# flock-lab/flock

Hardware: AMD Instinct MI355X
Metric: NEXMark rows/sec per node (q3 join, q5 agg) (higher is better)
Workload: dtype int32; 1 GPU; NEXMark q5 hopping(10,5) over 1087 s x 1000000 events/s per GPU; query=q5, input_rows_per_gpu=1000040000, windows_per_gpu=216, parallelism=one GPU, one process

## Files before the change

flock_amd/csrc/q5.hip:

```cpp
#include <algorithm>

#include "sort.hpp"

using namespace flockgpu;

namespace {

constexpr int kQ5Iters = 8;
constexpr int kQ5Tile = kBlock * 4 * kQ5Iters;
constexpr int kHist = 4096;
constexpr int kHistPad = 64;
constexpr int kSlots = kHist / 2;
constexpr int kSlotBits = 11;
static_assert(kSlots == (1 << kSlotBits), "slot bits");
constexpr int kLdsMaxProbe = 24;
constexpr uint32_t kFib = 0x9E3779B1u;
constexpr int kHotMin = 16;
constexpr int kMaxWinPanes = 8;
constexpr uint32_t kWideTile = 0x40000000u;

using u16x2 = unsigned short __attribute__((ext_vector_type(2)));
__device__ __forceinline__ u16x2 as_u16x2(uint32_t w) { return __builtin_bit_cast(u16x2, w); }
__device__ __forceinline__ u16x2 nonzero_u16x2(u16x2 c) {
    uint32_t r;
// ... 95 lines not shown
        const int32_t w = f.pane_win_idx[wi];
        table_add(f.tables + (size_t)w * f.cap, f.cap, (uint32_t)key, c, &f.tab_used[w], f.err);
    }
}

__device__ __forceinline__ void emit_pair16(int32_t even_key, uint32_t c0, uint32_t c1, const FlushArgs &f) {
    const uint64_t idx = (uint64_t)((int64_t)even_key - f.pane.base);
    if (idx < (uint64_t)f.pane.range) {
        __hip_atomic_fetch_add(&f.counters[(f.pane.cnt_off + idx) >> 1], c0 | (c1 << 16), __ATOMIC_RELAXED, __HIP_MEMORY_SCOPE_AGENT);
        return;
    }
    if (c0) emit_pair(even_key, c0, f);
    if (c1) emit_pair(even_key + 1, c1, f);
}

constexpr int kRangeBlocks = 2;
__global__ __launch_bounds__(kBlock) void q5_range_kernel(const int32_t *__restrict__ auction, int64_t n_rows,
                                                          const int64_t *__restrict__ seg_off, int32_t *__restrict__ rng) {
    __shared__ int32_t s_red[8];
    const int32_t pane = blockIdx.y;
    const int64_t sb = seg_off[2 * pane], se = seg_off[2 * pane + 1];
    const int64_t groups = (se - (sb & ~int64_t(3)) + 3) >> 2;
    const int64_t n_samples = (int64_t)kRangeBlocks * kBlock * 4;
    const int64_t stride = groups > n_samples ? groups / n_samples : 1;
    int32_t mn = 0x7fffffff, mx = (int32_t)0x80000000;
#pragma unroll
    for (int i = 0; i < 4; ++i) {
        const int64_t g = ((int64_t)(i * kRangeBlocks + blockIdx.x) * kBlock + threadIdx.x) * stride;
        const int64_t r0 = (sb & ~int64_t(3)) + g * 4;
        if (g < groups && r0 + 4 <= n_rows) {
            const int4 t = *reinterpret_cast<const int4 *>(auction + r0);
            const int32_t k[4] = {t.x, t.y, t.z, t.w};
#pragma unroll
            for (int j = 0; j < 4; ++j)
                if (r0 + j >= sb && r0 + j < se) {
                    mn = min(mn, k[j]);
                    mx = max(mx, k[j]);
                }
        }
    }
#pragma unroll
    for (int o = 32; o > 0; o >>= 1) {
        mn = min(mn, __shfl_xor(mn, o, 64));
        mx = max(mx, __shfl_xor(mx, o, 64));
    }
    if (lane_id() == 0) {
        s_red[threadIdx.x >> 6] = mn;
        s_red[4 + (threadIdx.x >> 6)] = mx;
    }
    __syncthreads();
    if (threadIdx.x == 0) {
        int32_t *o = rng + ((size_t)pane * kRangeBlocks + blockIdx.x) * 2;
        o[0] = min(min(s_red[0], s_red[1]), min(s_red[2], s_red[3]));
        o[1] = max(max(s_red[4], s_red[5]), max(s_red[6], s_red[7]));
    }
}

__host__ __device__ inline bool q5_pane_layout(int64_t lo, int64_t hi, int64_t *base, int64_t *range) {
    const int64_t span = hi - lo, margin = span / 16 > 4096 ? span / 16 : 4096;
    *base = (lo - margin) & ~int64_t(7);
    *range = ((hi + margin + 1 - *base) + 7) & ~int64_t(7);
    return *range < (int64_t(1) << 31);
}

struct LayoutArgs {
    const int32_t *rng;
    const int32_t *pane_win_ptr;
    const int64_t *seg_off;
    int32_t n_panes, n_win;
    uint64_t capacity, budget_bytes;
    PaneDesc *panes;
    WinDesc *wins;
    uint64_t *info;
};
__device__ __forceinline__ void q5_layout_block(const int32_t *__restrict__ rng, const int32_t *__restrict__ pane_win_ptr,
                                                const int64_t *__restrict__ seg_off, int32_t n_panes, int32_t n_win,
                                                uint64_t capacity, uint64_t budget_bytes, PaneDesc *__restrict__ panes,
                                                WinDesc *__restrict__ wins, uint64_t *__restrict__ info) {
    __shared__ uint64_t s_wave[kWavesPerBlock];
    __shared__ uint64_t s_carry;
    __shared__ int s_ok;
    const int lane = lane_id(), wave = threadIdx.x >> 6;
    if (threadIdx.x == 0) {
        s_carry = 0;
        s_ok = 1;
    }
    __syncthreads();
    for (int32_t p0 = 0; p0 < n_panes; p0 += kBlock) {
        const int32_t p = p0 + (int32_t)threadIdx.x;
        int64_t base = 0, range = 0;
        if (p < n_panes && pane_win_ptr[p + 1] != pane_win_ptr[p] && seg_off[2 * p + 1] > seg_off[2 * p]) {
            int32_t mn = 0x7fffffff, mx = (int32_t)0x80000000;
            for (int b = 0; b < kRangeBlocks; ++b) {
                mn = min(mn, rng[((size_t)p * kRangeBlocks + b) * 2]);
                mx = max(mx, rng[((size_t)p * kRangeBlocks + b) * 2 + 1]);
            }
            if (mn <= mx && !q5_pane_layout(mn, mx, &base, &range)) {
                s_ok = 0;
                range = 0;
            }
        }
        const uint64_t incl = wave_incl_scan_u64((uint64_t)range);
        if (lane == 63) s_wave[wave] = incl;
        __syncthreads();
        uint64_t off = s_carry + incl - (uint64_t)range;
        for (int v = 0; v < wave; ++v) off += s_wave[v];
        if (p < n_panes) panes[p] = PaneDesc{base, off, (uint32_t)range, 0};
        __syncthreads();
        if (threadIdx.x == kBlock - 1) s_carry = off + (uint64_t)range;
        __syncthreads();
    }
    const uint64_t cnt_total = s_carry;
    __syncthreads();
    uint64_t scan = 0;
    for (int32_t w = threadIdx.x; w < n_win; w += kBlock) {
        WinDesc d = wins[w];
// ... 15 lines not shown
                scan += (uint64_t)(hi - lo);
            }
        }
        wins[w] = d;
    }
    scan = wave_sum_u64(scan);
    if (lane == 0) s_wave[wave] = scan;
    __syncthreads();
    if (threadIdx.x == 0) {
        uint64_t scan_total = 0;
        for (int v = 0; v < kWavesPerBlock; ++v) scan_total += s_wave[v];
        const bool ok = s_ok && cnt_total <= capacity && cnt_total * 4 <= budget_bytes && scan_total * 4 <= 2 * budget_bytes;
        info[0] = cnt_total;
        info[1] = scan_total;
        info[2] = ok ? 1 : 0;
    }
}

__global__ __launch_bounds__(kBlock) void q5_clear_kernel(uint32_t *__restrict__ counters, uint64_t cnt_host,
                                                          uint64_t cnt_from, uint64_t *__restrict__ tables, uint64_t table_words,
                                                          uint64_t *__restrict__ meta, uint64_t meta_words, int32_t *__restrict__ slow_list,
                                                          uint32_t *__restrict__ block_max, uint64_t block_max_words, int c16, LayoutArgs lay,
                                                          const uint64_t *__restrict__ cnt_info) {
    if (lay.rng && blockIdx.x == 0) q5_layout_block(lay.rng, lay.pane_win_ptr, lay.seg_off, lay.n_panes, lay.n_win, lay.capacity, lay.budget_bytes, lay.panes, lay.wins, lay.info);
    uint64_t cnt = cnt_host;
    if (cnt_info) cnt = cnt_info[2] ? (cnt_info[0] < cnt_host ? cnt_info[0] : cnt_host) : 0;
    if (c16) cnt = (cnt + 1) / 2;
    const uint64_t i0 = (uint64_t)blockIdx.x * kBlock + threadIdx.x, stride = (uint64_t)gridDim.x * kBlock;
    const uint4 z = make_uint4(0, 0, 0, 0);
    for (uint64_t i = i0 + cnt_from / 4; i * 4 < cnt + 3; i += stride) {
        uint32_t *p = counters + i * 4;
        __builtin_nontemporal_store(0u, p);
        __builtin_nontemporal_store(0u, p + 1);
        __builtin_nontemporal_store(0u, p + 2);
        __builtin_nontemporal_store(0u, p + 3);
    }
    for (uint64_t i = i0; i * 2 < table_words; i += stride) {
        if (i * 2 + 1 < table_words) reinterpret_cast<uint4 *>(tables)[i] = z;
        else tables[i * 2] = 0;
    }
// ... 706 lines not shown
            uint64_t t = 0;
#pragma unroll
            for (int v = 0; v < kWavesPerBlock; ++v) t += s_groups[2][v];
            if (t) atomicAdd(&pane_sum[p], (unsigned long long)t);
        }
    }
}

constexpr int kFinishThreads = 1024;
constexpr uint32_t kFinishMax = 1024;
__global__ __launch_bounds__(kFinishThreads) void q5_finish_kernel(const uint64_t *__restrict__ meta, uint32_t n_meta, int32_t n_win, const uint64_t *__restrict__ info,
                                                                   const int32_t *__restrict__ slow_list, const int32_t *__restrict__ sel_win,
                                                                   const int32_t *__restrict__ sel_key, uint32_t out_cap, int32_t *__restrict__ out_auction,
                                                                   uint64_t *__restrict__ out_num, uint64_t *__restrict__ h_fin,
                                                                   const unsigned long long *__restrict__ pane_sum, const unsigned long long *__restrict__ tab_rows,
                                                                   const int64_t *__restrict__ seg_off, const int32_t *__restrict__ pane_win_ptr, int32_t n_panes) {
    __shared__ uint64_t s_k[kFinishMax];
    __shared__ uint32_t s_bad;
    const uint32_t *tail = reinterpret_cast<const uint32_t *>(meta + 2 * (size_t)n_win);
    const uint32_t n_sel = tail[0], err = tail[1];
    if (threadIdx.x == 0) s_bad = 0;
    __syncthreads();
    if (pane_sum && (!info || info[2]))
        for (int32_t p = threadIdx.x; p < n_panes; p += kFinishThreads)
            if (pane_win_ptr[p + 1] != pane_win_ptr[p] && pane_sum[p] + tab_rows[p] != (unsigned long long)(seg_off[2 * p + 1] - seg_off[2 * p])) s_bad = 1;
    __syncthreads();
    const uint32_t bad16 = s_bad;
    for (uint32_t i = threadIdx.x; i < n_meta; i += kFinishThreads) h_fin[i] = meta[i];
    if (threadIdx.x < 3) h_fin[n_meta + threadIdx.x] = info ? info[threadIdx.x] : 0;
    if (threadIdx.x == 3) h_fin[n_meta + 3] = (uint64_t)(uint32_t)slow_list[0] | ((uint64_t)bad16 << 32);
    const bool sortable = !err && !bad16 && n_sel <= kFinishMax && n_sel <= out_cap && (!info || info[2]);
    if (threadIdx.x == 4) h_fin[n_meta + 4] = sortable ? 1 : 0;
    int64_t *h_off = reinterpret_cast<int64_t *>(h_fin + n_meta + 5);
    if (!sortable) return;
    uint32_t p2 = 1;
    while (p2 < n_sel) p2 <<= 1;
    if (threadIdx.x < p2)
        s_k[threadIdx.x] = threadIdx.x < n_sel ? ((uint64_t)(uint32_t)sel_win[threadIdx.x] << 32) | ((uint32_t)sel_key[threadIdx.x] ^ 0x80000000u) : ~0ull;
    __syncthreads();
    for (uint32_t k = 2; k <= p2; k <<= 1)
        for (uint32_t j = k >> 1; j > 0; j >>= 1) {
            const uint32_t i = threadIdx.x, l = i ^ j;
            if (i < p2 && l > i) {
                const uint64_t a = s_k[i], b = s_k[l];
// ... 351 lines not shown
        now.insert(now.end(), idx.begin(), idx.end());
        if (sig != now) {
            std::copy(ptr.begin(), ptr.end(), h_ptr);
            std::copy(idx.begin(), idx.end(), h_idx);
            std::copy(role_a.begin(), role_a.end(), h_roles);
            std::copy(role_b.begin(), role_b.end(), h_roles + role_a.size());
            FG_HIP(ctx, hipMemcpyAsync(d_ptr, h_ptr, ptr.size() * sizeof(int32_t), hipMemcpyHostToDevice, ctx->stream));
            if (!idx.empty())
                FG_HIP(ctx, hipMemcpyAsync(d_idx, h_idx, idx.size() * sizeof(int32_t), hipMemcpyHostToDevice, ctx->stream));
            FG_HIP(ctx, hipMemcpyAsync(d_roles, h_roles, 2 * role_a.size() * sizeof(int32_t), hipMemcpyHostToDevice, ctx->stream));
            sig = now;
        }
    }

    int32_t *d_rng = nullptr, *h_rng = nullptr;
    const size_t n_rng = (size_t)2 * kRangeBlocks * std::max(n_panes, 1);
    FG_TRY(arena_get_t(ctx, "q5.pane_range", n_rng + 2, &d_rng));
    FG_TRY(pinned_get_t(ctx, "q5.pane_range", n_rng + 2, &h_rng));
    std::vector<PaneDesc> panes((size_t)std::max(n_panes, 1));
    std::vector<WinDesc> wins((size_t)std::max(n_win, 1));
    for (auto &p : panes) p = PaneDesc{0, 0, 0, 0};
    for (int w = 0; w < n_win; ++w) wins[w] = WinDesc{0, 0, win->win_pane_lo[w], win->win_pane_hi[w], 0};
    uint64_t cnt_total = 0, scan_total = 0;
    bool dense = st.n_tiles > 0 && n_win > 0 && max_win_panes <= kMaxWinPanes;
    std::vector<int64_t> &hint = ctx->host_i64[weight ? "q5.layout_hint.weighted" : "q5.layout_hint"];
    if (hint.size() != 3) hint.assign(3, 0);
    const uint64_t budget = std::max<uint64_t>(uint64_t(256) << 20, (uint64_t)covered_rows * 4 * 2);
    if (dense) {
        LaunchScope ls(ctx, "q5_range_kernel");
        hipLaunchKernelGGL(q5_range_kernel, dim3(kRangeBlocks, (unsigned)n_panes), dim3(kBlock), 0, ctx->stream, auction, rows, st.seg_off, d_rng);
    }
    FG_TRY(check_launch(ctx, "q5_range_kernel"));
    std::vector<int64_t> &wide_hint = ctx->host_i64["q5.wide_hint"];
    if (wide_hint.size() != 1) wide_hint.assign(1, 0);
    bool wide_mode = wide_hint[0] != 0 && !weight && !part && dense;
    bool wide_ran = false;
    bool speculate = dense && !part && hint[2] && hint[0] > 0 && !wide_mode;
    auto host_layout = [&]() -> int {
        FG_HIP(ctx, hipMemcpyAsync(h_rng, d_rng, sizeof(int32_t) * n_rng, hipMemcpyDeviceToHost, ctx->stream));
        FG_HIP(ctx, hipStreamSynchronize(ctx->stream));
        cnt_total = scan_total = 0;
        for (int p = 0; p < n_panes && dense; ++p) {
            if (ptr[p + 1] == ptr[p] || se[p] <= sb[p]) continue;
            int64_t lo = INT64_MAX, hi = INT64_MIN;
            for (int b = 0; b < kRangeBlocks; ++b) {
                lo = std::min<int64_t>(lo, h_rng[((size_t)p * kRangeBlocks + b) * 2]);
                hi = std::max<int64_t>(hi, h_rng[((size_t)p * kRangeBlocks + b) * 2 + 1]);
            }
            if (lo > hi) continue;
            int64_t base = 0, range = 0;
            if (!q5_pane_layout(lo, hi, &base, &range)) { dense = false; break; }
            panes[p] = PaneDesc{base, cnt_total, (uint32_t)range, 0};
            cnt_total += (uint64_t)range;
        }
        for (int w = 0; w < n_win && dense; ++w) {
            int64_t lo = INT64_MAX, hi = INT64_MIN;
            for (int p = win->win_pane_lo[w]; p < win->win_pane_hi[w]; ++p)
                if (panes[p].range) {
                    lo = std::min(lo, panes[p].base);
                    hi = std::max(hi, panes[p].base + (int64_t)panes[p].range);
                }
            if (lo >= hi) continue;
            if (hi - lo >= (int64_t(1) << 31)) { dense = false; break; }
            wins[w].base = lo;
            wins[w].range = (uint32_t)(hi - lo);
            scan_total += (uint64_t)(hi - lo);
        }
        if (dense && (cnt_total * 4 > budget || scan_total * 4 > 2 * budget)) dense = false;
        return FLOCKGPU_OK;
    };
    if (dense && !speculate) FG_TRY(host_layout());
    PaneDesc *d_panes = nullptr, *h_panes = nullptr;
    WinDesc *d_wins = nullptr, *h_wins = nullptr;
    FG_TRY(arena_get_t(ctx, "q5.panes", panes.size(), &d_panes));
    FG_TRY(pinned_get_t(ctx, "q5.panes", panes.size(), &h_panes));
    FG_TRY(arena_get_t(ctx, "q5.wins", wins.size(), &d_wins));
    FG_TRY(pinned_get_t(ctx, "q5.wins", wins.size(), &h_wins));
    uint64_t *d_info = nullptr, *h_info = nullptr;
    FG_TRY(arena_get_t(ctx, "q5.layout_info", 4, &d_info));
    FG_TRY(pinned_get_t(ctx, "q5.layout_info", 4, &h_info));
    auto upload_layout = [&]() -> int {
        if (!dense) {
            cnt_total = scan_total = 0;
            for (auto &p : panes) p = PaneDesc{0, 0, 0, 0};
            for (int w = 0; w < n_win; ++w) wins[w] = WinDesc{0, 0, win->win_pane_lo[w], win->win_pane_hi[w], 0};
        }
        std::copy(panes.begin(), panes.end(), h_panes);
        std::copy(wins.begin(), wins.end(), h_wins);
        ctx->host_i64["q5.wins_sig"].clear();
        FG_HIP(ctx, hipMemcpyAsync(d_panes, h_panes, panes.size() * sizeof(PaneDesc), hipMemcpyHostToDevice, ctx->stream));
        FG_HIP(ctx, hipMemcpyAsync(d_wins, h_wins, wins.size() * sizeof(WinDesc), hipMemcpyHostToDevice, ctx->stream));
        return FLOCKGPU_OK;
    };
    uint32_t *counters = nullptr;
    uint64_t capacity = 0;
    std::vector<int64_t> &preclean = ctx->host_i64["q5.preclean"];
    if (preclean.size() != 2) preclean.assign(2, 0);
    LayoutArgs lay{};
    uint64_t clean_upto = 0;
    const bool c16 = !weight && !part && !wide_mode && hop2 && ctx->host_i64["q5.no_c16"].empty();
    auto words_of = [&](uint64_t n_counters) -> uint64_t { return c16 ? (n_counters + 1) / 2 : n_counters; };
    if (speculate) {
        FG_TRY(arena_get_t(ctx, "q5.counters", (size_t)words_of((uint64_t)hint[0] + (uint64_t)hint[0] / 8) + 8, &counters));
        capacity = (ctx->arena["q5.counters"].cap / sizeof(uint32_t) - 8) * (c16 ? 2 : 1);
        if (preclean[0] == (int64_t)reinterpret_cast<uintptr_t>(counters)) clean_upto = (uint64_t)preclean[1];
        {
            std::vector<int64_t> &wsig = ctx->host_i64["q5.wins_sig"];
            std::vector<int64_t> wnow;
            wnow.reserve((size_t)2 * n_win + 2);
            wnow.push_back((int64_t)reinterpret_cast<uintptr_t>(d_wins));
            for (int w = 0; w < n_win; ++w) {
                wnow.push_back(win->win_pane_lo[w]);
                wnow.push_back(win->win_pane_hi[w]);
            }
            if (wsig != wnow) {
                std::copy(wins.begin(), wins.end(), h_wins);
                FG_HIP(ctx, hipMemcpyAsync(d_wins, h_wins, wins.size() * sizeof(WinDesc), hipMemcpyHostToDevice, ctx->stream));
                wsig = wnow;
            }
        }
// ... 18 lines not shown
    if (weight && n_panes > 0) {
        FG_TRY(arena_get_t(ctx, "q5.pane_weight", (size_t)n_panes + 1, &d_wsum));
        FG_TRY(pinned_get_t(ctx, "q5.pane_weight", (size_t)n_panes + 1, &h_wsum));
    }
    double rpg = ctx->q5_rows_per_group < 1.0 ? 1.0 : ctx->q5_rows_per_group;
    uint64_t cap64 = dense ? 1024 : std::max<uint64_t>(1024, (uint64_t)((double)max_win_rows / rpg * 2.0) + 64);
    uint32_t out_cap = 1u << 16;
    std::vector<int32_t> h_win, h_key;
    uint32_t n_sel = 0;
    const int32_t *sel_win = nullptr, *sel_key = nullptr;
    bool fin_sorted = false;
    const int64_t *fin_off = nullptr;
    const int32_t *fin_auction = nullptr;
    const uint64_t *fin_num = nullptr;
    uint32_t h_slow_count = 0;
    for (int attempt = 0;; ++attempt) {
        if (attempt > 8 || cap64 >= (uint64_t(1) << 31))
            return fail(ctx, FLOCKGPU_ERR_CAPACITY, "q5: hash table capacity %llu still overflows", (unsigned long long)cap64);
        const uint32_t cap = (uint32_t)cap64;
        const uint64_t *spec_info = speculate ? d_info : nullptr;
        uint64_t *tables = nullptr;
        FG_TRY(arena_get_t(ctx, "q5.tables", (size_t)cap * std::max(n_win, 1), &tables));
        int32_t *o_win = nullptr, *o_key = nullptr, *slow_list = nullptr;
        FG_TRY(arena_get_t(ctx, "q5.sel_win", out_cap, &o_win));
        FG_TRY(arena_get_t(ctx, "q5.sel_key", out_cap, &o_key));
        FG_TRY(arena_get_t(ctx, "q5.slow_list", (size_t)st.n_tiles + 2, &slow_list));
        const uint64_t per_win = n_win > 0 ? std::max<uint64_t>(cap, scan_total / n_win / 4) : cap;
        const bool pane_walk = hop2;
        const uint64_t per_pane = n_panes > 0 ? std::max<uint64_t>(cap, cnt_total / (uint64_t)n_panes / 4) : cap;
        const int hop2_blocks = c16 ? 16 : 32;
        const unsigned gx = (unsigned)std::min<int64_t>(std::max<int64_t>(div_up((int64_t)(pane_walk ? per_pane : per_win), kBlock * 2), 1), pane_walk ? hop2_blocks : 64);
        uint32_t *block_max = nullptr;
        const uint64_t n_block_max = (uint64_t)gx * std::max(n_win, 1) * (pane_walk ? 2 : 1);
        FG_TRY(arena_get_t(ctx, "q5.block_max", (size_t)n_block_max, &block_max));
        {
            const uint64_t clear_words = std::max<uint64_t>({words_of(speculate ? capacity : cnt_total), (uint64_t)cap * n_win, (uint64_t)n_meta_all, n_block_max});
            const unsigned cg = (unsigned)std::max<int64_t>(1, std::min<int64_t>(div_up((int64_t)clear_words / 4 + 1, kBlock), (int64_t)ctx->num_cus * 16));
            {
                LaunchScope ls(ctx, "q5_clear_kernel");
                hipLaunchKernelGGL(q5_clear_kernel, dim3(cg), dim3(kBlock), 0, ctx->stream, counters, speculate ? capacity : cnt_total,
                                   (attempt == 0 && speculate) ? (clean_upto & ~uint64_t(3)) : uint64_t(0), tables, (uint64_t)cap * n_win, d_meta, (uint64_t)n_meta_all,
                                   slow_list, block_max, n_block_max, c16 ? 1 : 0, speculate ? lay : LayoutArgs{}, (const uint64_t *)nullptr);
                if (speculate) clean_upto = std::max(clean_upto, words_of(capacity));
            }
            FG_TRY(check_launch(ctx, "q5_clear_kernel"));
        }
        if (d_wsum) FG_HIP(ctx, hipMemsetAsync(d_wsum, 0, sizeof(unsigned long long) * (size_t)n_panes, ctx->stream));
        uint32_t nd = 0;
        if (wide_mode && dense) {
            uint32_t max_range = 0;
            for (int p = 0; p < n_panes; ++p) max_range = std::max(max_range, panes[(size_t)p].range);
            nd = (uint32_t)div_up((int64_t)max_range, int64_t(1) << kPartShift) + 1;
        }
        const bool wide = wide_mode && dense && nd >= 2 && nd <= (uint32_t)kPartMaxDigits && st.n_tiles > 0 && n_win > 0;
        wide_ran = wide;
        uint32_t *d_sample = nullptr, *h_sample = nullptr;
        FG_TRY(arena_get_t(ctx, "q5.part_sample", 4, &d_sample));
// ... 20 lines not shown
                LaunchScope ls(ctx, "q5_bucket_count_kernel");
                hipLaunchKernelGGL(q5_bucket_count_kernel, dim3(nd, (unsigned)n_panes), dim3(kBlock), 0, ctx->stream, part_keys, part_low, st4, d_panes, d_ptr, d_idx, nd,
                                   off_mat, counters, tables, cap, d_used, d_err);
            }
            FG_TRY(check_launch(ctx, "q5_bucket_count_kernel"));
            FG_HIP(ctx, hipMemcpyAsync(h_sample, d_sample, 2 * sizeof(uint32_t), hipMemcpyDeviceToHost, ctx->stream));
        } else if (st.n_tiles > 0 && n_win > 0) {
            {
                LaunchScope ls(ctx, "q5_count_kernel");
                hipLaunchKernelGGL(weight ? q5_count_kernel<true> : q5_count_kernel<false>, dim3((unsigned)st.n_tiles), dim3(kBlock), 0,
                                   ctx->stream, auction, weight, st, d_panes, d_ptr, d_idx, counters, tables, cap, d_used, d_err,
                                   slow_list, spec_info, d_wsum, c16 ? 1 : 0, c16 ? d_tab_rows : (unsigned long long *)nullptr);
            }
            FG_TRY(check_launch(ctx, "q5_count_kernel"));
            if (d_wsum) FG_HIP(ctx, hipMemcpyAsync(h_wsum, d_wsum, sizeof(unsigned long long) * (size_t)n_panes, hipMemcpyDeviceToHost, ctx->stream));
            {
                LaunchScope ls(ctx, "q5_count_slow_kernel");
                const unsigned gs = (unsigned)std::min<int64_t>(st.n_tiles, (int64_t)ctx->num_cus * 8);
                hipLaunchKernelGGL(weight ? q5_count_slow_kernel<true> : q5_count_slow_kernel<false>, dim3(gs), dim3(kBlock), 0,
                                   ctx->stream, auction, weight, st, d_panes, d_ptr, d_idx, counters, tables, cap, d_used, d_err,
                                   slow_list, spec_info, c16 ? 1 : 0, c16 ? d_tab_rows : (unsigned long long *)nullptr);
            }
            FG_TRY(check_launch(ctx, "q5_count_slow_kernel"));
        }
        if (part) {
            const int64_t tab0 = ((int64_t)cnt_total + 3) & ~int64_t(3);
            std::vector<int64_t> xb((size_t)2 * n_win), xe((size_t)2 * n_win);
            for (int w = 0; w < n_win; ++w) {
                xb[2 * w] = (int64_t)panes[w].cnt_off;
                xe[2 * w] = (int64_t)panes[w].cnt_off + (int64_t)panes[w].range;
                xb[2 * w + 1] = tab0 + (int64_t)w * cap;
// ... 73 lines not shown
            }
            FG_TRY(check_launch(ctx, "q5_select_kernel"));
        }
        constexpr uint32_t kSpecWinners = 4096;
        uint64_t *h_fin = nullptr;
        int32_t *fin_a = nullptr;
        uint64_t *fin_n = nullptr;
        FG_TRY(pinned_get_t(ctx, "q5.finish", n_meta + 8 + (size_t)n_win + 2, &h_fin));
        FG_TRY(arena_get_t(ctx, "q5.out_auction", (size_t)kFinishMax + 1, &fin_a));
        FG_TRY(arena_get_t(ctx, "q5.out_num", (size_t)kFinishMax + 1, &fin_n));
        const bool poll = !d_wsum && !wide;
        if (poll) pinned_pending(h_fin, (int)(n_meta + 5 + (size_t)n_win + 1));
        {
            LaunchScope ls(ctx, "q5_finish_kernel");
            hipLaunchKernelGGL(q5_finish_kernel, dim3(1), dim3(kFinishThreads), 0, ctx->stream, d_meta, (uint32_t)n_meta, n_win, spec_info, slow_list, o_win, o_key, out_cap,
                               fin_a, fin_n, h_fin, c16 && pane_walk ? d_pane_sum : (const unsigned long long *)nullptr, d_tab_rows, st.seg_off, d_ptr, n_panes);
        }
        FG_TRY(check_launch(ctx, "q5_finish_kernel"));
        if (speculate && dense) {
            LaunchScope ls(ctx, "q5_clear_kernel");
            const unsigned cg = (unsigned)std::max<int64_t>(1, std::min<int64_t>(div_up((int64_t)words_of(cnt_total) / 4 + 1, kBlock), (int64_t)ctx->num_cus * 16));
            hipLaunchKernelGGL(q5_clear_kernel, dim3(cg), dim3(kBlock), 0, ctx->stream, counters, capacity, uint64_t(0), (uint64_t *)nullptr,
                               uint64_t(0), (uint64_t *)nullptr, uint64_t(0), slow_list, (uint32_t *)nullptr, uint64_t(0), c16 ? 1 : 0, LayoutArgs{}, d_info);
        }
        FG_TRY(check_launch(ctx, "q5_clear_kernel"));
        if (poll) {
            FG_TRY(wait_pinned(ctx, h_fin, (int)(n_meta + 5)));
            if (h_fin[n_meta + 4]) FG_TRY(wait_pinned(ctx, h_fin + n_meta + 5, n_win + 1));
        } else
            FG_HIP(ctx, hipStreamSynchronize(ctx->stream));
        std::copy(h_fin, h_fin + n_meta, h_meta);
        if (speculate) std::copy(h_fin + n_meta, h_fin + n_meta + 3, h_info);
        h_slow_count = (uint32_t)h_fin[n_meta + 3];
        if (h_fin[n_meta + 3] >> 32) {
            ctx->host_i64["q5.no_c16"].assign(1, 1);
            return q5_run(ctx, auction, weight, rows, win, out, part);
        }
        fin_sorted = h_fin[n_meta + 4] != 0;
        fin_off = reinterpret_cast<const int64_t *>(h_fin + n_meta + 5);
        if (speculate) {
            if (!h_info[2]) {
                speculate = false;
                hint[2] = 0;
                FG_TRY(host_layout());
                FG_TRY(upload_layout());
                FG_TRY(arena_get_t(ctx, "q5.counters", (size_t)words_of(cnt_total) + 8, &counters));
                cap64 = dense ? 1024 : std::max<uint64_t>(1024, (uint64_t)((double)max_win_rows / rpg * 2.0) + 64);
                --attempt;
                continue;
            }
            cnt_total = h_info[0];
            scan_total = h_info[1];
        }
        if (h_wsum) {
            for (int w = 0; w < n_win; ++w) {
                unsigned long long tot = 0;
                for (int p = win->win_pane_lo[w]; p < win->win_pane_hi[w]; ++p) tot += h_wsum[p];
                if (tot >= (1ull << 32))
                    return fail(ctx, FLOCKGPU_ERR_UNSUPPORTED, "q5 weighted: the counts of window %d add up to %llu >= 2^32 (32-bit counters)", w, tot);
            }
        }
        const uint32_t *tail = reinterpret_cast<const uint32_t *>(h_meta + 2 * n_win);
        n_sel = tail[0];
        if (tail[1]) {
            cap64 *= 4;
            continue;
        }
// ... 4 lines not shown
        h_win.resize(n_sel);
        h_key.resize(n_sel);
        if (fin_sorted) {
            fin_auction = fin_a;
            fin_num = fin_n;
        } else if (n_sel <= kSpecWinners) {
            FG_HIP(ctx, hipMemcpyAsync(h_win.data(), o_win, sizeof(int32_t) * n_sel, hipMemcpyDeviceToHost, ctx->stream));
            FG_HIP(ctx, hipMemcpyAsync(h_key.data(), o_key, sizeof(int32_t) * n_sel, hipMemcpyDeviceToHost, ctx->stream));
            FG_HIP(ctx, hipStreamSynchronize(ctx->stream));
        } else {
            sel_win = o_win;
            sel_key = o_key;
        }
        break;
    }
    hint[0] = (int64_t)cnt_total;
    hint[1] = (int64_t)scan_total;
    hint[2] = dense ? 1 : 0;
    if (!weight && !part) {
        uint32_t *h_sample = nullptr;
        FG_TRY(pinned_get_t(ctx, "q5.part_sample", 4, &h_sample));
        if (wide_mode && !wide_ran) wide_hint[0] = 0;
        else if (wide_mode && h_sample[0]) wide_hint[0] = (uint64_t)h_sample[1] * 4 >= (uint64_t)h_sample[0] * 3 ? 0 : 1;
        else if (!wide_mode && dense && st.n_tiles > 64) wide_hint[0] = (int64_t)h_slow_count * 4 > (int64_t)st.n_tiles ? 1 : 0;
    }
    {
        double best = 1e30;
        for (int w = 0; w < n_win; ++w) {
            const int64_t rows = win->pane_row_offsets[win->win_pane_hi[w]] - win->pane_row_offsets[win->win_pane_lo[w]];
            const uint64_t g = h_meta[n_win + w];
            if (g) best = std::min(best, (double)rows / (double)g);
        }
        if (best < 1e30) ctx->q5_rows_per_group = best;
    }
    std::vector<int64_t> &offs = ctx->host_i64["q5.win_out_offsets"];
    std::vector<uint64_t> &wmax = ctx->host_u64["q5.win_max"], &wgrp = ctx->host_u64["q5.win_groups"];
    offs.assign((size_t)n_win + 1, 0);
    wmax.assign(h_meta, h_meta + n_win);
    wgrp.assign(h_meta + n_win, h_meta + 2 * n_win);
// ... 16 lines not shown
        FG_TRY(key_min_max(ctx, sel_key, n_sel, d_mm));
        FG_HIP(ctx, hipMemcpyAsync(h_mm, d_mm, 2 * sizeof(int32_t), hipMemcpyDeviceToHost, ctx->stream));
        FG_HIP(ctx, hipStreamSynchronize(ctx->stream));
        int bits = 1, wbits = 1;
        while (bits < 32 && (((uint64_t)((int64_t)h_mm[1] - (int64_t)h_mm[0])) >> bits)) ++bits;
        while (wbits < 31 && ((uint32_t)n_win >> wbits)) ++wbits;
        FG_TRY(radix_sort_pairs(ctx, "q5.ord_key", sel_key, nullptr, n_sel, h_mm[0], bits, &k1, &v1));
        FG_TRY(arena_get_t(ctx, "q5.ord_win_in", (size_t)n_sel + 4, &w_in));
        FG_TRY(gather_i32(ctx, sel_win, reinterpret_cast<const int32_t *>(v1), n_sel, w_in));
        FG_TRY(radix_sort_pairs(ctx, "q5.ord_win", w_in, v1, n_sel, 0, wbits, &w2, &v2));
        FG_TRY(arena_get_t(ctx, "q5.out_auction", (size_t)n_sel + 1, &d_oa));
        FG_TRY(arena_get_t(ctx, "q5.out_num", (size_t)n_sel + 1, &d_on));
        FG_TRY(arena_get_t(ctx, "q5.ord_off", (size_t)n_win + 2, &d_off));
        FG_TRY(pinned_get_t(ctx, "q5.ord_off", (size_t)n_win + 2, &h_off));
        FG_TRY(gather_i32(ctx, sel_key, reinterpret_cast<const int32_t *>(v2), n_sel, d_oa));
        hipLaunchKernelGGL(q5_winner_num_kernel, dim3((unsigned)div_up((int64_t)n_sel, kBlock)), dim3(kBlock), 0, ctx->stream, w2,
                           d_meta, (int64_t)n_sel, d_on);
        FG_TRY(check_launch(ctx, "q5_winner_num_kernel"));
        FG_TRY(sorted_key_offsets(ctx, w2, n_sel, n_win, d_off));
        FG_HIP(ctx, hipMemcpyAsync(h_off, d_off, sizeof(int64_t) * ((size_t)n_win + 1), hipMemcpyDeviceToHost, ctx->stream));
        FG_HIP(ctx, hipStreamSynchronize(ctx->stream));
        offs.assign(h_off, h_off + n_win + 1);
        out->auction = d_oa;
        out->num = d_on;
        out->win_out_offsets = offs.data();
        out->win_max = wmax.data();
        out->win_groups = wgrp.data();
        out->rows = n_sel;
        return FLOCKGPU_OK;
    }
// ... 19 lines not shown
    FG_TRY(arena_get_t(ctx, "q5.out_auction", (size_t)n_sel + 1, &d_oa));
    FG_TRY(arena_get_t(ctx, "q5.out_num", (size_t)n_sel + 1, &d_on));
    if (n_sel) {
        FG_HIP(ctx, hipMemcpyAsync(d_oa, h_oa, sizeof(int32_t) * n_sel, hipMemcpyHostToDevice, ctx->stream));
        FG_HIP(ctx, hipMemcpyAsync(d_on, h_on, sizeof(uint64_t) * n_sel, hipMemcpyHostToDevice, ctx->stream));
    }
    out->auction = d_oa;
    out->num = d_on;
    out->win_out_offsets = offs.data();
    out->win_max = wmax.data();
    out->win_groups = wgrp.data();
    out->rows = n_sel;
    }
    if (speculate && dense && cnt_total > 0) {
        preclean[0] = (int64_t)reinterpret_cast<uintptr_t>(counters);
        preclean[1] = (int64_t)std::max<uint64_t>(clean_upto, words_of(cnt_total));
    }
    return FLOCKGPU_OK;
}

namespace flockgpu {

int q5_partial_by_tile(flockgpu_ctx *ctx, const flockgpu_bid_cols *bid, const flockgpu_windows *win, Q5TilePartial *out) {
    *out = Q5TilePartial{};
    FG_TRY(check_windows(ctx, win, bid->rows, "q5 partial"));
    if (bid->rows > 0 && !bid->auction) return fail(ctx, FLOCKGPU_ERR_INVALID, "q5 partial: null auction column");
    if (reinterpret_cast<uintptr_t>(bid->auction) & 15) return fail(ctx, FLOCKGPU_ERR_UNSUPPORTED, "q5: auction column must be 16-byte aligned");
    if (bid->rows >= (int64_t(1) << 31)) return fail(ctx, FLOCKGPU_ERR_UNSUPPORTED, "q5 partial: more than 2^31 rows per call");
    FG_HIP(ctx, hipSetDevice(ctx->device));
    const int n_panes = win->n_panes;
    std::vector<char> used((size_t)std::max(n_panes, 1), 0);
// ... 83 lines not shown
```

Baseline: 1351 billion rows/s.

## Use fixed per-pane counter slots with in-kernel layout and skip redundant clears

The range kernel now runs one 1024-thread block per pane, computes each pane's layout descriptor on the device, and assigns fixed-size counter slots sized from a remembered max pane range. On steady repeated calls this lets the path skip the full clear/layout kernel. The post-finish clear runs per pane, and the slow-path count kernel is skipped unless slow tiles were seen recently. The goal is to cut per-call launch, clear and layout overhead. The cost is much more complex state tracking across calls, with a retry if skipped slow work turns out to be needed.

```diff
diff --git a/flock_amd/csrc/q5.hip b/flock_amd/csrc/q5.hip
--- a/flock_amd/csrc/q5.hip
+++ b/flock_amd/csrc/q5.hip
@@ -133,23 +133,44 @@
     if (c1) emit_pair(even_key + 1, c1, f);
 }
 
+__host__ __device__ inline bool q5_pane_layout(int64_t lo, int64_t hi, int64_t *base, int64_t *range) {
+    const int64_t span = hi - lo, margin = span / 16 > 4096 ? span / 16 : 4096;
+    *base = (lo - margin) & ~int64_t(7);
+    *range = ((hi + margin + 1 - *base) + 7) & ~int64_t(7);
+    return *range < (int64_t(1) << 31);
+}
+
 constexpr int kRangeBlocks = 2;
-__global__ __launch_bounds__(kBlock) void q5_range_kernel(const int32_t *__restrict__ auction, int64_t n_rows,
-                                                          const int64_t *__restrict__ seg_off, int32_t *__restrict__ rng) {
-    __shared__ int32_t s_red[8];
+constexpr int kRangeThreads = 1024;
+constexpr int kRangeSamples = kRangeBlocks * kBlock * 4 / kRangeThreads;
+__global__ __launch_bounds__(kRangeThreads) void q5_range_kernel(const int32_t *__restrict__ auction, int64_t n_rows,
+                                                                 const int64_t *__restrict__ seg_off, int32_t *__restrict__ rng,
+                                                                 PaneDesc *__restrict__ panes_out, const int32_t *__restrict__ pane_win_ptr,
+                                                                 uint64_t slot, uint64_t *__restrict__ info) {
+    constexpr int kWaves = kRangeThreads / 64;
+    __shared__ int32_t s_red[2 * kWaves];
     const int32_t pane = blockIdx.y;
     const int64_t sb = seg_off[2 * pane], se = seg_off[2 * pane + 1];
+    const bool used = panes_out && threadIdx.x == 0 ? pane_win_ptr[pane + 1] != pane_win_ptr[pane] : false;
     const int64_t groups = (se - (sb & ~int64_t(3)) + 3) >> 2;
     const int64_t n_samples = (int64_t)kRangeBlocks * kBlock * 4;
     const int64_t stride = groups > n_samples ? groups / n_samples : 1;
     int32_t mn = 0x7fffffff, mx = (int32_t)0x80000000;
-#pragma unroll
-    for (int i = 0; i < 4; ++i) {
-        const int64_t g = ((int64_t)(i * kRangeBlocks + blockIdx.x) * kBlock + threadIdx.x) * stride;
+    int4 t[kRangeSamples];
+    bool have[kRangeSamples];
+#pragma unroll
+    for (int i = 0; i < kRangeSamples; ++i) {
+        const int64_t g = ((int64_t)i * kRangeThreads + threadIdx.x) * stride;
         const int64_t r0 = (sb & ~int64_t(3)) + g * 4;
-        if (g < groups && r0 + 4 <= n_rows) {
-            const int4 t = *reinterpret_cast<const int4 *>(auction + r0);
-            const int32_t k[4] = {t.x, t.y, t.z, t.w};
+        have[i] = g < groups && r0 + 4 <= n_rows;
+        t[i] = have[i] ? *reinterpret_cast<const int4 *>(auction + r0) : make_int4(0, 0, 0, 0);
+    }
+#pragma unroll
+    for (int i = 0; i < kRangeSamples; ++i) {
+        const int64_t g = ((int64_t)i * kRangeThreads + threadIdx.x) * stride;
+        const int64_t r0 = (sb & ~int64_t(3)) + g * 4;
+        if (have[i]) {
+            const int32_t k[4] = {t[i].x, t[i].y, t[i].z, t[i].w};
 #pragma unroll
             for (int j = 0; j < 4; ++j)
                 if (r0 + j >= sb && r0 + j < se) {
@@ -165,21 +186,26 @@
     }
     if (lane_id() == 0) {
         s_red[threadIdx.x >> 6] = mn;
-        s_red[4 + (threadIdx.x >> 6)] = mx;
+        s_red[kWaves + (threadIdx.x >> 6)] = mx;
     }
     __syncthreads();
     if (threadIdx.x == 0) {
-        int32_t *o = rng + ((size_t)pane * kRangeBlocks + blockIdx.x) * 2;
-        o[0] = min(min(s_red[0], s_red[1]), min(s_red[2], s_red[3]));
-        o[1] = max(max(s_red[4], s_red[5]), max(s_red[6], s_red[7]));
-    }
-}
-
-__host__ __device__ inline bool q5_pane_layout(int64_t lo, int64_t hi, int64_t *base, int64_t *range) {
-    const int64_t span = hi - lo, margin = span / 16 > 4096 ? span / 16 : 4096;
-    *base = (lo - margin) & ~int64_t(7);
-    *range = ((hi + margin + 1 - *base) + 7) & ~int64_t(7);
-    return *range < (int64_t(1) << 31);
+#pragma unroll
+        for (int v = 0; v < kWaves; ++v) {
+            mn = min(mn, s_red[v]);
+            mx = max(mx, s_red[kWaves + v]);
+        }
+        rng[(size_t)pane * 2] = mn;
+        rng[(size_t)pane * 2 + 1] = mx;
+        if (panes_out) {
+            int64_t base = 0, range = 0;
+            if (used && se > sb && mn <= mx && (!q5_pane_layout(mn, mx, &base, &range) || (uint64_t)range > slot)) {
+                info[2] = 0;
+                range = 0;
+            }
+            panes_out[pane] = PaneDesc{base, (uint64_t)pane * slot, (uint32_t)range, 0};
+        }
+    }
 }
 
 struct LayoutArgs {
@@ -199,26 +225,25 @@
     __shared__ uint64_t s_wave[kWavesPerBlock];
     __shared__ uint64_t s_carry;
     __shared__ int s_ok;
+    __shared__ uint32_t s_max_range;
     const int lane = lane_id(), wave = threadIdx.x >> 6;
     if (threadIdx.x == 0) {
         s_carry = 0;
         s_ok = 1;
+        s_max_range = 0;
     }
     __syncthreads();
     for (int32_t p0 = 0; p0 < n_panes; p0 += kBlock) {
         const int32_t p = p0 + (int32_t)threadIdx.x;
         int64_t base = 0, range = 0;
         if (p < n_panes && pane_win_ptr[p + 1] != pane_win_ptr[p] && seg_off[2 * p + 1] > seg_off[2 * p]) {
-            int32_t mn = 0x7fffffff, mx = (int32_t)0x80000000;
-            for (int b = 0; b < kRangeBlocks; ++b) {
-                mn = min(mn, rng[((size_t)p * kRangeBlocks + b) * 2]);
-                mx = max(mx, rng[((size_t)p * kRangeBlocks + b) * 2 + 1]);
-            }
+            const int32_t mn = rng[(size_t)p * 2], mx = rng[(size_t)p * 2 + 1];
             if (mn <= mx && !q5_pane_layout(mn, mx, &base, &range)) {
                 s_ok = 0;
                 range = 0;
             }
         }
+        if (range) atomicMax(&s_max_range, (uint32_t)range);
         const uint64_t incl = wave_incl_scan_u64((uint64_t)range);
         if (lane == 63) s_wave[wave] = incl;
         __syncthreads();
@@ -264,6 +289,7 @@
         info[0] = cnt_total;
         info[1] = scan_total;
         info[2] = ok ? 1 : 0;
+        info[3] = s_max_range;
     }
 }
 
@@ -271,9 +297,27 @@
                                                           uint64_t cnt_from, uint64_t *__restrict__ tables, uint64_t table_words,
                                                           uint64_t *__restrict__ meta, uint64_t meta_words, int32_t *__restrict__ slow_list,
                                                           uint32_t *__restrict__ block_max, uint64_t block_max_words, int c16, LayoutArgs lay,
-                                                          const uint64_t *__restrict__ cnt_info) {
+                                                          const uint64_t *__restrict__ cnt_info, const PaneDesc *__restrict__ pane_clean,
+                                                          uint64_t *__restrict__ layout_info) {
     if (lay.rng && blockIdx.x == 0) q5_layout_block(lay.rng, lay.pane_win_ptr, lay.seg_off, lay.n_panes, lay.n_win, lay.capacity, lay.budget_bytes, lay.panes, lay.wins, lay.info);
     uint64_t cnt = cnt_host;
+    if (pane_clean) {
+        const PaneDesc pd = pane_clean[blockIdx.y];
+        if (pd.cnt_off + (uint64_t)pd.range <= cnt_host) {
+            uint32_t *mine = counters + (c16 ? pd.cnt_off / 2 : pd.cnt_off);
+            const uint64_t words = c16 ? pd.range / 2 : pd.range;
+            for (uint64_t i = (uint64_t)blockIdx.x * kBlock + threadIdx.x; i * 4 < words; i += (uint64_t)gridDim.x * kBlock) {
+                uint32_t *p = mine + i * 4;
+                __builtin_nontemporal_store(0u, p);
+                __builtin_nontemporal_store(0u, p + 1);
+                __builtin_nontemporal_store(0u, p + 2);
+                __builtin_nontemporal_store(0u, p + 3);
+            }
+        }
+        if (blockIdx.y != 0) return;
+        if (blockIdx.x == 0 && threadIdx.x == 0) layout_info[2] = 1;
+        cnt = 0;
+    } else
     if (cnt_info) cnt = cnt_info[2] ? (cnt_info[0] < cnt_host ? cnt_info[0] : cnt_host) : 0;
     if (c16) cnt = (cnt + 1) / 2;
     const uint64_t i0 = (uint64_t)blockIdx.x * kBlock + threadIdx.x, stride = (uint64_t)gridDim.x * kBlock;
@@ -1010,7 +1054,8 @@
                                                                    const int32_t *__restrict__ sel_key, uint32_t out_cap, int32_t *__restrict__ out_auction,
                                                                    uint64_t *__restrict__ out_num, uint64_t *__restrict__ h_fin,
                                                                    const unsigned long long *__restrict__ pane_sum, const unsigned long long *__restrict__ tab_rows,
-                                                                   const int64_t *__restrict__ seg_off, const int32_t *__restrict__ pane_win_ptr, int32_t n_panes) {
+                                                                   const int64_t *__restrict__ seg_off, const int32_t *__restrict__ pane_win_ptr, int32_t n_panes,
+                                                                   int pane_report) {
     __shared__ uint64_t s_k[kFinishMax];
     __shared__ uint32_t s_bad;
     const uint32_t *tail = reinterpret_cast<const uint32_t *>(meta + 2 * (size_t)n_win);
@@ -1023,7 +1068,7 @@
     __syncthreads();
     const uint32_t bad16 = s_bad;
     for (uint32_t i = threadIdx.x; i < n_meta; i += kFinishThreads) h_fin[i] = meta[i];
-    if (threadIdx.x < 3) h_fin[n_meta + threadIdx.x] = info ? info[threadIdx.x] : 0;
+    if (threadIdx.x < 3) h_fin[n_meta + threadIdx.x] = info ? info[pane_report && threadIdx.x == 1 ? 3 : threadIdx.x] : 0;
     if (threadIdx.x == 3) h_fin[n_meta + 3] = (uint64_t)(uint32_t)slow_list[0] | ((uint64_t)bad16 << 32);
     const bool sortable = !err && !bad16 && n_sel <= kFinishMax && n_sel <= out_cap && (!info || info[2]);
     if (threadIdx.x == 4) h_fin[n_meta + 4] = sortable ? 1 : 0;
@@ -1405,7 +1450,7 @@
     }
 
     int32_t *d_rng = nullptr, *h_rng = nullptr;
-    const size_t n_rng = (size_t)2 * kRangeBlocks * std::max(n_panes, 1);
+    const size_t n_rng = (size_t)2 * std::max(n_panes, 1);
     FG_TRY(arena_get_t(ctx, "q5.pane_range", n_rng + 2, &d_rng));
     FG_TRY(pinned_get_t(ctx, "q5.pane_range", n_rng + 2, &h_rng));
     std::vector<PaneDesc> panes((size_t)std::max(n_panes, 1));
@@ -1415,29 +1460,30 @@
     uint64_t cnt_total = 0, scan_total = 0;
     bool dense = st.n_tiles > 0 && n_win > 0 && max_win_panes <= kMaxWinPanes;
     std::vector<int64_t> &hint = ctx->host_i64[weight ? "q5.layout_hint.weighted" : "q5.layout_hint"];
-    if (hint.size() != 3) hint.assign(3, 0);
+    if (hint.size() != 4) hint.assign(4, 0);
     const uint64_t budget = std::max<uint64_t>(uint64_t(256) << 20, (uint64_t)covered_rows * 4 * 2);
-    if (dense) {
-        LaunchScope ls(ctx, "q5_range_kernel");
-        hipLaunchKernelGGL(q5_range_kernel, dim3(kRangeBlocks, (unsigned)n_panes), dim3(kBlock), 0, ctx->stream, auction, rows, st.seg_off, d_rng);
-    }
-    FG_TRY(check_launch(ctx, "q5_range_kernel"));
     std::vector<int64_t> &wide_hint = ctx->host_i64["q5.wide_hint"];
     if (wide_hint.size() != 1) wide_hint.assign(1, 0);
     bool wide_mode = wide_hint[0] != 0 && !weight && !part && dense;
     bool wide_ran = false;
     bool speculate = dense && !part && hint[2] && hint[0] > 0 && !wide_mode;
+    PaneDesc *d_panes = nullptr, *h_panes = nullptr;
+    uint64_t *d_info = nullptr, *h_info = nullptr;
+    auto launch_range = [&](PaneDesc *po, uint64_t slot) -> int {
+        {
+            LaunchScope ls(ctx, "q5_range_kernel");
+            hipLaunchKernelGGL(q5_range_kernel, dim3(1, (unsigned)n_panes), dim3(kRangeThreads), 0, ctx->stream, auction, rows, st.seg_off, d_rng, po, (const int32_t *)d_ptr, slot, d_info);
+        }
+        return check_launch(ctx, "q5_range_kernel");
+    };
+    if (dense && !speculate) FG_TRY(launch_range(nullptr, 0));
     auto host_layout = [&]() -> int {
         FG_HIP(ctx, hipMemcpyAsync(h_rng, d_rng, sizeof(int32_t) * n_rng, hipMemcpyDeviceToHost, ctx->stream));
         FG_HIP(ctx, hipStreamSynchronize(ctx->stream));
         cnt_total = scan_total = 0;
         for (int p = 0; p < n_panes && dense; ++p) {
             if (ptr[p + 1] == ptr[p] || se[p] <= sb[p]) continue;
-            int64_t lo = INT64_MAX, hi = INT64_MIN;
-            for (int b = 0; b < kRangeBlocks; ++b) {
-                lo = std::min<int64_t>(lo, h_rng[((size_t)p * kRangeBlocks + b) * 2]);
-                hi = std::max<int64_t>(hi, h_rng[((size_t)p * kRangeBlocks + b) * 2 + 1]);
-            }
+            const int64_t lo = h_rng[(size_t)p * 2], hi = h_rng[(size_t)p * 2 + 1];
             if (lo > hi) continue;
             int64_t base = 0, range = 0;
             if (!q5_pane_layout(lo, hi, &base, &range)) { dense = false; break; }
@@ -1461,13 +1507,11 @@
         return FLOCKGPU_OK;
     };
     if (dense && !speculate) FG_TRY(host_layout());
-    PaneDesc *d_panes = nullptr, *h_panes = nullptr;
     WinDesc *d_wins = nullptr, *h_wins = nullptr;
     FG_TRY(arena_get_t(ctx, "q5.panes", panes.size(), &d_panes));
     FG_TRY(pinned_get_t(ctx, "q5.panes", panes.size(), &h_panes));
     FG_TRY(arena_get_t(ctx, "q5.wins", wins.size(), &d_wins));
     FG_TRY(pinned_get_t(ctx, "q5.wins", wins.size(), &h_wins));
-    uint64_t *d_info = nullptr, *h_info = nullptr;
     FG_TRY(arena_get_t(ctx, "q5.layout_info", 4, &d_info));
     FG_TRY(pinned_get_t(ctx, "q5.layout_info", 4, &h_info));
     auto upload_layout = [&]() -> int {
@@ -1491,10 +1535,23 @@
     uint64_t clean_upto = 0;
     const bool c16 = !weight && !part && !wide_mode && hop2 && ctx->host_i64["q5.no_c16"].empty();
     auto words_of = [&](uint64_t n_counters) -> uint64_t { return c16 ? (n_counters + 1) / 2 : n_counters; };
+    const bool pane_mode = speculate && hop2 && !weight;
+    std::vector<int64_t> left_clean;
+    left_clean.swap(ctx->host_i64["q5.left_clean"]);
+    uint64_t slot = 0;
     if (speculate) {
-        FG_TRY(arena_get_t(ctx, "q5.counters", (size_t)words_of((uint64_t)hint[0] + (uint64_t)hint[0] / 8) + 8, &counters));
+        uint64_t want = (uint64_t)hint[0] + (uint64_t)hint[0] / 8;
+        if (pane_mode && hint[3] > 0) {
+            const uint64_t slot_want = (((uint64_t)hint[3] + (uint64_t)hint[3] / 8) + 7) & ~uint64_t(7);
+            if (slot_want * (uint64_t)n_panes * 4 <= budget) want = std::max(want, slot_want * (uint64_t)n_panes);
+        }
+        FG_TRY(arena_get_t(ctx, "q5.counters", (size_t)words_of(want) + 8, &counters));
         capacity = (ctx->arena["q5.counters"].cap / sizeof(uint32_t) - 8) * (c16 ? 2 : 1);
         if (preclean[0] == (int64_t)reinterpret_cast<uintptr_t>(counters)) clean_upto = (uint64_t)preclean[1];
+        if (pane_mode && hint[3] > 0) {
+            slot = (capacity / (uint64_t)n_panes) & ~uint64_t(7);
+            if (slot < (uint64_t)hint[3] || slot * (uint64_t)n_panes * 4 > budget || slot >= (uint64_t(1) << 31)) slot = 0;
+        }
         {
             std::vector<int64_t> &wsig = ctx->host_i64["q5.wins_sig"];
             std::vector<int64_t> wnow;
@@ -1543,6 +1600,15 @@
     const int32_t *fin_auction = nullptr;
     const uint64_t *fin_num = nullptr;
     uint32_t h_slow_count = 0;
+    uint64_t max_pane_range = (uint64_t)hint[3];
+    std::vector<int64_t> &slow_hint = ctx->host_i64["q5.slow_hint"];
+    if (slow_hint.size() != 1) slow_hint.assign(1, 0);
+    bool slow_skipped = false;
+    std::vector<int64_t> clean_now;
+    bool steady = false;
+    bool slotted = false;
+    bool pane_cleaned = false;
+    bool slow_needed = false;
     for (int attempt = 0;; ++attempt) {
         if (attempt > 8 || cap64 >= (uint64_t(1) << 31))
             return fail(ctx, FLOCKGPU_ERR_CAPACITY, "q5: hash table capacity %llu still overflows", (unsigned long long)cap64);
@@ -1562,14 +1628,21 @@
         uint32_t *block_max = nullptr;
         const uint64_t n_block_max = (uint64_t)gx * std::max(n_win, 1) * (pane_walk ? 2 : 1);
         FG_TRY(arena_get_t(ctx, "q5.block_max", (size_t)n_block_max, &block_max));
-        {
+        clean_now.assign({(int64_t)reinterpret_cast<uintptr_t>(counters), (int64_t)capacity, c16 ? 1 : 0, (int64_t)reinterpret_cast<uintptr_t>(tables), (int64_t)cap, n_win, n_panes,
+                          (int64_t)reinterpret_cast<uintptr_t>(d_meta), (int64_t)n_meta_all, (int64_t)reinterpret_cast<uintptr_t>(block_max), (int64_t)n_block_max,
+                          (int64_t)reinterpret_cast<uintptr_t>(slow_list), (int64_t)reinterpret_cast<uintptr_t>(d_info), (int64_t)reinterpret_cast<uintptr_t>(d_panes)});
+        steady = attempt == 0 && pane_mode && speculate && slot > 0 && left_clean == clean_now && clean_upto >= words_of(slot * (uint64_t)n_panes);
+        if (attempt == 0 && speculate) FG_TRY(launch_range(steady ? d_panes : nullptr, slot));
+        if (steady) slotted = true;
+        if (!steady) {
             const uint64_t clear_words = std::max<uint64_t>({words_of(speculate ? capacity : cnt_total), (uint64_t)cap * n_win, (uint64_t)n_meta_all, n_block_max});
             const unsigned cg = (unsigned)std::max<int64_t>(1, std::min<int64_t>(div_up((int64_t)clear_words / 4 + 1, kBlock), (int64_t)ctx->num_cus * 16));
             {
                 LaunchScope ls(ctx, "q5_clear_kernel");
                 hipLaunchKernelGGL(q5_clear_kernel, dim3(cg), dim3(kBlock), 0, ctx->stream, counters, speculate ? capacity : cnt_total,
                                    (attempt == 0 && speculate) ? (clean_upto & ~uint64_t(3)) : uint64_t(0), tables, (uint64_t)cap * n_win, d_meta, (uint64_t)n_meta_all,
-                                   slow_list, block_max, n_block_max, c16 ? 1 : 0, speculate ? lay : LayoutArgs{}, (const uint64_t *)nullptr);
+                                   slow_list, block_max, n_block_max, c16 ? 1 : 0, speculate && !slotted ? lay : LayoutArgs{}, (const uint64_t *)nullptr, (const PaneDesc *)nullptr,
+                                   (uint64_t *)nullptr);
                 if (speculate) clean_upto = std::max(clean_upto, words_of(capacity));
             }
             FG_TRY(check_launch(ctx, "q5_clear_kernel"));
@@ -1620,7 +1693,8 @@
             }
             FG_TRY(check_launch(ctx, "q5_count_kernel"));
             if (d_wsum) FG_HIP(ctx, hipMemcpyAsync(h_wsum, d_wsum, sizeof(unsigned long long) * (size_t)n_panes, hipMemcpyDeviceToHost, ctx->stream));
-            {
+            slow_skipped = speculate && !weight && !slow_needed && slow_hint[0] == 0;
+            if (!slow_skipped) {
                 LaunchScope ls(ctx, "q5_count_slow_kernel");
                 const unsigned gs = (unsigned)std::min<int64_t>(st.n_tiles, (int64_t)ctx->num_cus * 8);
                 hipLaunchKernelGGL(weight ? q5_count_slow_kernel<true> : q5_count_slow_kernel<false>, dim3(gs), dim3(kBlock), 0,
@@ -1724,14 +1798,25 @@
         {
             LaunchScope ls(ctx, "q5_finish_kernel");
             hipLaunchKernelGGL(q5_finish_kernel, dim3(1), dim3(kFinishThreads), 0, ctx->stream, d_meta, (uint32_t)n_meta, n_win, spec_info, slow_list, o_win, o_key, out_cap,
-                               fin_a, fin_n, h_fin, c16 && pane_walk ? d_pane_sum : (const unsigned long long *)nullptr, d_tab_rows, st.seg_off, d_ptr, n_panes);
+                               fin_a, fin_n, h_fin, c16 && pane_walk ? d_pane_sum : (const unsigned long long *)nullptr, d_tab_rows, st.seg_off, d_ptr, n_panes,
+                               pane_mode && speculate ? 1 : 0);
         }
         FG_TRY(check_launch(ctx, "q5_finish_kernel"));
-        if (speculate && dense) {
+        pane_cleaned = false;
+        if (speculate && dense && pane_mode) {
+            LaunchScope ls(ctx, "q5_clear_kernel");
+            const uint64_t pane_words = words_of(slotted ? slot : cnt_total / (uint64_t)n_panes + 1);
+            const unsigned cgx = (unsigned)std::max<int64_t>(1, std::min<int64_t>(div_up((int64_t)pane_words / 4 + 1, kBlock), div_up((int64_t)ctx->num_cus * 16, n_panes)));
+            hipLaunchKernelGGL(q5_clear_kernel, dim3(cgx, (unsigned)n_panes), dim3(kBlock), 0, ctx->stream, counters, capacity, uint64_t(0), (uint64_t *)nullptr,
+                               uint64_t(0), d_meta, (uint64_t)n_meta_all, slow_list, block_max, n_block_max, c16 ? 1 : 0, LayoutArgs{}, (const uint64_t *)nullptr,
+                               (const PaneDesc *)d_panes, d_info);
+            pane_cleaned = true;
+        } else if (speculate && dense) {
             LaunchScope ls(ctx, "q5_clear_kernel");
             const unsigned cg = (unsigned)std::max<int64_t>(1, std::min<int64_t>(div_up((int64_t)words_of(cnt_total) / 4 + 1, kBlock), (int64_t)ctx->num_cus * 16));
             hipLaunchKernelGGL(q5_clear_kernel, dim3(cg), dim3(kBlock), 0, ctx->stream, counters, capacity, uint64_t(0), (uint64_t *)nullptr,
-                               uint64_t(0), (uint64_t *)nullptr, uint64_t(0), slow_list, (uint32_t *)nullptr, uint64_t(0), c16 ? 1 : 0, LayoutArgs{}, d_info);
+                               uint64_t(0), (uint64_t *)nullptr, uint64_t(0), slow_list, (uint32_t *)nullptr, uint64_t(0), c16 ? 1 : 0, LayoutArgs{}, d_info, (const PaneDesc *)nullptr,
+                               (uint64_t *)nullptr);
         }
         FG_TRY(check_launch(ctx, "q5_clear_kernel"));
         if (poll) {
@@ -1742,6 +1827,10 @@
         std::copy(h_fin, h_fin + n_meta, h_meta);
         if (speculate) std::copy(h_fin + n_meta, h_fin + n_meta + 3, h_info);
         h_slow_count = (uint32_t)h_fin[n_meta + 3];
+        if (slow_skipped && h_slow_count) {
+            slow_needed = true;
+            continue;
+        }
         if (h_fin[n_meta + 3] >> 32) {
             ctx->host_i64["q5.no_c16"].assign(1, 1);
             return q5_run(ctx, auction, weight, rows, win, out, part);
@@ -1759,8 +1848,14 @@
                 --attempt;
                 continue;
             }
-            cnt_total = h_info[0];
-            scan_total = h_info[1];
+            {
+                cnt_total = h_info[0];
+                scan_total = h_info[1];
+                if (pane_mode) {
+                    max_pane_range = h_info[1];
+                    scan_total = 2 * cnt_total;
+                }
+            }
         }
         if (h_wsum) {
             for (int w = 0; w < n_win; ++w) {
@@ -1795,6 +1890,11 @@
         }
         break;
     }
+    if (!speculate) {
+        max_pane_range = 0;
+        for (const PaneDesc &p : panes) max_pane_range = std::max<uint64_t>(max_pane_range, p.range);
+    }
+    hint[3] = (int64_t)max_pane_range;
     hint[0] = (int64_t)cnt_total;
     hint[1] = (int64_t)scan_total;
     hint[2] = dense ? 1 : 0;
@@ -1804,6 +1904,8 @@
         if (wide_mode && !wide_ran) wide_hint[0] = 0;
         else if (wide_mode && h_sample[0]) wide_hint[0] = (uint64_t)h_sample[1] * 4 >= (uint64_t)h_sample[0] * 3 ? 0 : 1;
         else if (!wide_mode && dense && st.n_tiles > 64) wide_hint[0] = (int64_t)h_slow_count * 4 > (int64_t)st.n_tiles ? 1 : 0;
+        constexpr int64_t kSlowKeep = 1;
+        if (!wide_mode) slow_hint[0] = h_slow_count ? kSlowKeep : std::max<int64_t>(slow_hint[0] - 1, 0);
     }
     {
         double best = 1e30;
@@ -1850,6 +1952,8 @@
         FG_TRY(arena_get_t(ctx, "q5.ord_off", (size_t)n_win + 2, &d_off));
         FG_TRY(pinned_get_t(ctx, "q5.ord_off", (size_t)n_win + 2, &h_off));
         FG_TRY(gather_i32(ctx, sel_key, reinterpret_cast<const int32_t *>(v2), n_sel, d_oa));
+        if (pane_cleaned)
+            FG_HIP(ctx, hipMemcpyAsync(d_meta, h_meta, sizeof(uint64_t) * (size_t)n_win, hipMemcpyHostToDevice, ctx->stream));
         hipLaunchKernelGGL(q5_winner_num_kernel, dim3((unsigned)div_up((int64_t)n_sel, kBlock)), dim3(kBlock), 0, ctx->stream, w2,
                            d_meta, (int64_t)n_sel, d_on);
         FG_TRY(check_launch(ctx, "q5_winner_num_kernel"));
@@ -1899,7 +2003,10 @@
     }
     if (speculate && dense && cnt_total > 0) {
         preclean[0] = (int64_t)reinterpret_cast<uintptr_t>(counters);
-        preclean[1] = (int64_t)std::max<uint64_t>(clean_upto, words_of(cnt_total));
+        preclean[1] = (int64_t)std::max<uint64_t>(clean_upto, words_of(slotted ? slot * (uint64_t)n_panes : cnt_total));
+        bool tables_used = reinterpret_cast<const uint32_t *>(h_meta + 2 * n_win)[1] != 0;
+        for (int w = 0; w < n_win && !tables_used; ++w) tables_used = reinterpret_cast<const uint32_t *>(h_meta + 2 * n_win)[2 + w] != 0;
+        if (pane_cleaned && !tables_used) ctx->host_i64["q5.left_clean"] = clean_now;
     }
     return FLOCKGPU_OK;
 }
```

New measurement: 1351 billion rows/s. About the same (-0.0%).
